# 0xMiden/miden-vm

Hardware: AMD Instinct MI355X
Metric: trace rows/sec proved (2^20-row trace, 96-bit sec) (higher is better)
Workload: dtype u64 (Goldilocks field, p = 2^64 - 2^32 + 1); 1 GPU; full proof of miden:20:51:8 (DummyMidenAir 2^20 x 51 + 8 EF aux), 96-bit production PCS params (blowup 8, FRI arity 4, 27 queries, PoW 4/12/16), Poseidon2 LMCS; trace resident in HBM, transcript on host; log_trace_rows=20, main_width=51, aux_width_ef=8, log_blowup=3, proof_bytes=137697, parallelism=1 GPU

## Files before the change

miden-vm_amd/csrc/deep.hip:

```cpp
#include "gl.cuh"
#include "kernels.hpp"

__global__ __launch_bounds__(256) void k_bary_weights(const u64* tw, int log_n, u64 g, e2 y0, e2 y1, u64* w0, u64* w1) {
  const size_t n = (size_t)1 << log_n;
  const size_t base = (size_t)blockIdx.x * 1024 + threadIdx.x;
  const size_t half = n >> 1;
  u64 xs[4], nrm[8], pre[8];
  e2 den[8];
#pragma unroll
  for (int k = 0; k < 4; k++) {
    size_t r = base + (size_t)k * 256;
    u64 x = 0;
    if (r < n) x = gl_mul(g, half ? (r < half ? tw[r] : gl_neg(tw[r - half])) : 1);
    xs[k] = x;
    den[2 * k] = e2_sub(y0, e2_make(x));
    den[2 * k + 1] = e2_sub(y1, e2_make(x));
  }
  u64 run = 1;
#pragma unroll
  for (int k = 0; k < 8; k++) {
    nrm[k] = gl_sub(gl_sqr(den[k].c0), gl_mul7(gl_sqr(den[k].c1)));
    pre[k] = run;
    run = gl_mul(run, nrm[k]);
  }
  u64 inv = gl_inv(run);
#pragma unroll
  for (int k = 7; k >= 0; k--) {
    u64 ni = gl_mul(inv, pre[k]);
    inv = gl_mul(inv, nrm[k]);
    size_t r = base + (size_t)(k >> 1) * 256;
    if (r < n) {
      u64 s = gl_mul(ni, xs[k >> 1]);
      u64* w = (k & 1) ? w1 : w0;
      w[2 * r] = gl_mul(den[k].c0, s);
      w[2 * r + 1] = gl_mul(gl_neg(den[k].c1), s);
    }
  }
}

static constexpr int OOD_ROWS_PER_BLOCK = 8192;
__global__ __launch_bounds__(256) void k_ood_partial(const u64* lde, int log_n, int log_blowup, const u64* w0, const u64* w1,
                                                     u64* partial, unsigned chunks) {
  __shared__ u64 red[4][256];
  const size_t n = (size_t)1 << log_n;
  const size_t col = blockIdx.y, chunk = blockIdx.x;
  const u64* f = lde + ((col << log_blowup) << log_n);
  const size_t r0 = chunk * OOD_ROWS_PER_BLOCK;
  const size_t r1 = r0 + OOD_ROWS_PER_BLOCK < n ? r0 + OOD_ROWS_PER_BLOCK : n;
  e2 a0 = e2_make(0), a1 = e2_make(0);
  for (size_t r = r0 + threadIdx.x; r < r1; r += 256) {
    u64 v = f[r];
    a0 = e2_add(a0, e2_mulf(e2{w0[2 * r], w0[2 * r + 1]}, v));
    a1 = e2_add(a1, e2_mulf(e2{w1[2 * r], w1[2 * r + 1]}, v));
  }
  red[0][threadIdx.x] = a0.c0; red[1][threadIdx.x] = a0.c1; red[2][threadIdx.x] = a1.c0; red[3][threadIdx.x] = a1.c1;
  __syncthreads();
  for (int s = 128; s > 0; s >>= 1) {
    if ((int)threadIdx.x < s) {
#pragma unroll
      for (int k = 0; k < 4; k++) red[k][threadIdx.x] = gl_add(red[k][threadIdx.x], red[k][threadIdx.x + s]);
    }
    __syncthreads();
  }
  if (threadIdx.x < 4) partial[(col * chunks + chunk) * 4 + threadIdx.x] = red[threadIdx.x][0];
}

void deep_ood_eval_batch(mh_ctx* c, std::vector<OodJob>& jobs, int log_blowup) {
  struct Weights {
    int log_n;
    size_t coset0;
    e2 y0, y1;
    DevBuf w0, w1;
  };
  std::vector<std::unique_ptr<Weights>> weights;
  struct Slot {
    size_t off = 0, ncol = 0;
    unsigned chunks = 0;
  };
  std::vector<Slot> slots(jobs.size());
  size_t total = 0;
  for (size_t k = 0; k < jobs.size(); k++) {
    OodJob& j = jobs[k];
    const LdeMatrix& m = *j.m;
    if (j.col_end > m.width) j.col_end = m.width;
    j.out0.assign(m.width, e2_make(0));
    j.out1.assign(m.width, e2_make(0));
    if (j.col_begin >= j.col_end) continue;
    const size_t n = (size_t)1 << m.log_n;
    slots[k].ncol = j.col_end - j.col_begin;
    slots[k].chunks = (unsigned)((n + OOD_ROWS_PER_BLOCK - 1) / OOD_ROWS_PER_BLOCK);
    slots[k].off = total;
    total += slots[k].ncol * slots[k].chunks * 4;
  }
  if (!total) return;
  DevBuf partial(total * 8), one;
  for (size_t k = 0; k < jobs.size(); k++) {
    if (!slots[k].ncol) continue;
    const OodJob& j = jobs[k];
    const LdeMatrix& m = *j.m;
    const int log_n = m.log_n;
    const size_t n = (size_t)1 << log_n;
    const u64 g = gl_mul(gl_lde_shift(log_n + log_blowup), gl_pow(gl_two_adic_generator(log_n + log_blowup), m.coset0));
    const u64* tw = log_n ? c->twiddles(log_n, false) : nullptr;
    if (!tw) {
      if (!one.p) {
        one.alloc(8);
        u64 v = 1;
        c->h2d(one.p, &v, 8);
      }
      tw = one.u();
    }
    ProfScope ps(c, "deep_ood_eval", (double)n * 8.0 * slots[k].ncol + 64.0 * n);
    Weights* w = nullptr;
    for (auto& cand : weights)
      if (cand->log_n == log_n && cand->coset0 == m.coset0 && e2_eq(cand->y0, j.y0) && e2_eq(cand->y1, j.y1)) w = cand.get();
    if (!w) {
      weights.emplace_back(new Weights{log_n, m.coset0, j.y0, j.y1, DevBuf(n * 16), DevBuf(n * 16)});
      w = weights.back().get();
      MH_LAUNCH(k_bary_weights, dim3((unsigned)((n + 1023) / 1024)), dim3(256), 0, c->stream, tw, log_n, g, j.y0, j.y1, w->w0.u(), w->w1.u());
    }
    MH_LAUNCH(k_ood_partial, dim3(slots[k].chunks, (unsigned)slots[k].ncol), dim3(256), 0, c->stream,
              m.lde.u() + ((j.col_begin << m.log_cosets) << log_n), log_n, m.log_cosets, w->w0.u(), w->w1.u(), partial.u() + slots[k].off,
              slots[k].chunks);
  }
  std::vector<u64> host(total);
  c->d2h(host.data(), partial.p, total * 8);
  for (size_t k = 0; k < jobs.size(); k++) {
    if (!slots[k].ncol) continue;
    OodJob& j = jobs[k];
    const LdeMatrix& m = *j.m;
    const int log_n = m.log_n;
    const size_t n = (size_t)1 << log_n;
    const u64 g = gl_mul(gl_lde_shift(log_n + log_blowup), gl_pow(gl_two_adic_generator(log_n + log_blowup), m.coset0));
    const u64 g_inv = gl_inv(g), n_inv = gl_inv((u64)n % GL_P);
    const e2 s0 = e2_mulf(e2_sub(e2_exp_pow2(e2_mulf(j.y0, g_inv), log_n), e2_make(1)), n_inv);
    const e2 s1 = e2_mulf(e2_sub(e2_exp_pow2(e2_mulf(j.y1, g_inv), log_n), e2_make(1)), n_inv);
    for (size_t col = 0; col < slots[k].ncol; col++) {
      e2 a0 = e2_make(0), a1 = e2_make(0);
      for (unsigned ch = 0; ch < slots[k].chunks; ch++) {
        const u64* p = host.data() + slots[k].off + (col * slots[k].chunks + ch) * 4;
        a0 = e2_add(a0, e2{p[0], p[1]});
        a1 = e2_add(a1, e2{p[2], p[3]});
      }
      j.out0[j.col_begin + col] = e2_mul(a0, s0);
      j.out1[j.col_begin + col] = e2_mul(a1, s1);
    }
  }
}
void deep_ood_eval_matrix(mh_ctx* c, const LdeMatrix& m, int log_blowup, e2 y0, e2 y1, std::vector<e2>& out0, std::vector<e2>& out1,
                          size_t col_begin, size_t col_end) {
  std::vector<OodJob> jobs(1);
  jobs[0].m = &m; jobs[0].y0 = y0; jobs[0].y1 = y1; jobs[0].col_begin = col_begin; jobs[0].col_end = col_end;
  deep_ood_eval_batch(c, jobs, log_blowup);
  out0.swap(jobs[0].out0);
  out1.swap(jobs[0].out1);
}

static constexpr int DEEP_MAX_MATS = 128;
static constexpr unsigned DEEP_FLUSH = 128;
#ifndef DEEP_UNROLL
#define DEEP_UNROLL 2
#endif
#ifndef DEEP_PTS_N
#define DEEP_PTS_N 1
#endif
static constexpr int DEEP_PTS = DEEP_PTS_N;
struct DeepMat {
  const u64* lde;
  u32 width, coef_off;
  int log_n;
};
struct DeepArgs {
  DeepMat m[DEEP_MAX_MATS];
  int n_mats, log_n, log_blowup;
  const u64* negc;
  const u64* tw;
  const u64* coset_x;
  e2 z0, z1, fred0, fred1, beta;
  u64* out;
};

__global__ __launch_bounds__(256) void k_deep_assemble(DeepArgs a) {
  const size_t N = (size_t)1 << a.log_n;
  const size_t j = blockIdx.y;
  const size_t base = (size_t)blockIdx.x * (256 * DEEP_PTS) + threadIdx.x;
  size_t r[DEEP_PTS];
#pragma unroll
  for (int k = 0; k < DEEP_PTS; k++) r[k] = base + (size_t)k * 256;
  e2 neg[DEEP_PTS];
  u64 w[DEEP_PTS][2][6];
#pragma unroll
  for (int k = 0; k < DEEP_PTS; k++) {
    neg[k] = e2_make(0);
#pragma unroll
    for (int e = 0; e < 2; e++)
#pragma unroll
      for (int i = 0; i < 6; i++) w[k][e][i] = 0;
  }
  auto flush = [&]() {
    const u64 C[6] = {1ULL, 1ULL << 22, 1ULL << 44, 1ULL << 32, 1ULL << 54, GL_EPS << 12};
#pragma unroll
    for (int k = 0; k < DEEP_PTS; k++) {
      u64 s0 = w[k][0][0], s1 = w[k][1][0];
#pragma unroll
      for (int i = 1; i < 6; i++) {
        s0 = gl_add(s0, gl_mul(w[k][0][i], C[i]));
        s1 = gl_add(s1, gl_mul(w[k][1][i], C[i]));
      }
      neg[k] = e2_add(neg[k], e2{s0, s1});
#pragma unroll
      for (int e = 0; e < 2; e++)
#pragma unroll
        for (int i = 0; i < 6; i++) w[k][e][i] = 0;
    }
  };
  u32 pending = 0;
#pragma unroll 1
  for (int mi = 0; mi < a.n_mats; mi++) {
    const DeepMat m = a.m[mi];
    const size_t nm_mask = ((size_t)1 << m.log_n) - 1;
    const u64* colp = m.lde + (j << m.log_n);
    const size_t cstride = (size_t)1 << (m.log_n + a.log_blowup);
#pragma unroll DEEP_UNROLL
    for (u32 cidx = 0; cidx < m.width; cidx++) {
      const u64 cf0 = a.negc[2 * (m.coef_off + cidx)], cf1 = a.negc[2 * (m.coef_off + cidx) + 1];
      u32 al[2][3];
#pragma unroll
      for (int i = 0; i < 3; i++) {
        al[0][i] = (u32)(cf0 >> (22 * i)) & 0x3FFFFFu;
        al[1][i] = (u32)(cf1 >> (22 * i)) & 0x3FFFFFu;
      }
#pragma unroll
      for (int k = 0; k < DEEP_PTS; k++) {
        if (r[k] < N) {
          const u64 v = colp[r[k] & nm_mask];
          const u32 v0 = (u32)v, v1 = (u32)(v >> 32);
#pragma unroll
          for (int e = 0; e < 2; e++) {
            w[k][e][0] += (u64)al[e][0] * v0;
            w[k][e][1] += (u64)al[e][1] * v0;
            w[k][e][2] += (u64)al[e][2] * v0;
            w[k][e][3] += (u64)al[e][0] * v1;
            w[k][e][4] += (u64)al[e][1] * v1;
            w[k][e][5] += (u64)al[e][2] * v1;
          }
        }
      }
      colp += cstride;
      if (++pending == DEEP_FLUSH) {
        flush();
        pending = 0;
      }
    }
  }
  flush();
  const size_t half = N >> 1;
  const u64 cx = a.coset_x[j];
  e2 den[2 * DEEP_PTS];
  u64 nrm[2 * DEEP_PTS], pre[2 * DEEP_PTS];
#pragma unroll
  for (int k = 0; k < DEEP_PTS; k++) {
    u64 x = 0;
    if (r[k] < N) x = gl_mul(cx, half ? (r[k] < half ? a.tw[r[k]] : gl_neg(a.tw[r[k] - half])) : 1);
    den[2 * k] = e2_sub(a.z0, e2_make(x));
    den[2 * k + 1] = e2_sub(a.z1, e2_make(x));
  }
  u64 run = 1;
#pragma unroll
  for (int k = 0; k < 2 * DEEP_PTS; k++) {
    nrm[k] = gl_sub(gl_sqr(den[k].c0), gl_mul7(gl_sqr(den[k].c1)));
    pre[k] = run;
    run = gl_mul(run, nrm[k]);
  }
  u64 inv = gl_inv(run);
  e2 qinv[2 * DEEP_PTS];
#pragma unroll
  for (int k = 2 * DEEP_PTS - 1; k >= 0; k--) {
    u64 ni = gl_mul(inv, pre[k]);
    inv = gl_mul(inv, nrm[k]);
    qinv[k] = e2{gl_mul(den[k].c0, ni), gl_mul(gl_neg(den[k].c1), ni)};
  }
#pragma unroll
  for (int k = 0; k < DEEP_PTS; k++) {
    if (r[k] < N) {
      e2 v = e2_mul(qinv[2 * k], e2_add(a.fred0, neg[k]));
      v = e2_add(v, e2_mul(e2_mul(a.beta, qinv[2 * k + 1]), e2_add(a.fred1, neg[k])));
      ulonglong2* o = reinterpret_cast<ulonglong2*>(a.out + 2 * ((j << a.log_n) + r[k]));
      *o = make_ulonglong2(v.c0, v.c1);
    }
  }
}

void deep_assemble(mh_ctx* c, const std::vector<const LdeMatrix*>& mats, const std::vector<u32>& coef_off, int log_n, int log_blowup,
                   const std::vector<e2>& negc, e2 z0, e2 z1, e2 fred0, e2 fred1, e2 beta, u64* out) {
  MH_REQUIRE(mats.size() <= (size_t)DEEP_MAX_MATS, "too many committed matrices for one DEEP pass");
  const int lbl = mats[0]->log_cosets;
  const size_t coset0 = mats[0]->coset0;
  for (auto* m : mats) MH_REQUIRE(m->log_cosets == lbl && m->coset0 == coset0, "internal: matrices cover different cosets");
  const size_t N = (size_t)1 << log_n, B = (size_t)1 << lbl;
  const int L = log_n + log_blowup;
  std::vector<u64> blob;
  for (e2 v : negc) { blob.push_back(v.c0); blob.push_back(v.c1); }
  const size_t o_cx = blob.size();
  const u64 g = gl_lde_shift(L), wK = gl_two_adic_generator(L);
  u64 x = gl_mul(g, gl_pow(wK, coset0));
  for (size_t j = 0; j < B; j++) {
    blob.push_back(x);
    x = gl_mul(x, wK);
  }
  DevBuf dblob(blob.size() * 8), one;
  c->h2d(dblob.p, blob.data(), blob.size() * 8);
  const u64* tw = log_n ? c->twiddles(log_n, false) : nullptr;
  if (!tw) {
    one.alloc(8);
    u64 v = 1;
    c->h2d(one.p, &v, 8);
    tw = one.u();
  }
  DeepArgs a{};
  double bytes = 16.0 * N * B;
  for (size_t i = 0; i < mats.size(); i++) {
    a.m[i] = DeepMat{mats[i]->lde.u(), (u32)mats[i]->width, coef_off[i], mats[i]->log_n};
    bytes += 8.0 * (double)mats[i]->width * (double)(((size_t)1 << mats[i]->log_n) << lbl);
  }
  a.n_mats = (int)mats.size();
  a.log_n = log_n; a.log_blowup = lbl;
  a.negc = dblob.u(); a.tw = tw; a.coset_x = dblob.u() + o_cx;
  a.z0 = z0; a.z1 = z1; a.fred0 = fred0; a.fred1 = fred1; a.beta = beta; a.out = out;
  {
    ProfScope ps(c, "deep_assemble", bytes);
    MH_LAUNCH(k_deep_assemble, dim3((unsigned)((N + 256 * DEEP_PTS - 1) / (256 * DEEP_PTS)), (unsigned)B), dim3(256), 0, c->stream, a);
  }
  HIP_CHECK(hipStreamSynchronize(c->stream));
}
```

miden-vm_amd/csrc/kernels.hpp:

```cpp
#pragma once
#include "../../include/midenhip.h"
#include "ctx.hpp"
#include <functional>
#include <vector>

void launch_transpose_rm_to_cm(mh_ctx* c, const u64* in_rowmajor, u64* out_colmajor, size_t n, size_t w, hipStream_t stream = nullptr);
void ntt_inverse_dif_inplace(mh_ctx* c, u64* cols, size_t n_cols, int log_n);
void ntt_inverse_dif(mh_ctx* c, const u64* src, u64* dst, size_t n_cols, int log_n);
void ntt_forward_cosets(mh_ctx* c, const u64* coef_br, size_t n_cols, int log_n, const std::vector<u64>& bases, u64* out, size_t out_col_stride = 0,
                        size_t group_cols = 0);
void lde_columns(mh_ctx* c, const u64* cols_in, size_t n_cols, int log_n, u64 in_shift, const std::vector<u64>& out_shifts,
                 u64* out, u64* scratch);
void lde_coefficients(mh_ctx* c, const u64* cols_in, size_t n_cols, int log_n, u64* coef_br);
void lde_forward_group(mh_ctx* c, const u64* coef_br, size_t n_cols, int log_n, u64 in_shift, const std::vector<u64>& group_shifts,
                       u64* out, size_t out_col_stride);

struct mh_trace {
  mh_ctx* ctx;
  int log_n;
  size_t width;
  DevBuf cols;
  hipEvent_t ready = nullptr;
  mutable DevBuf staging;
  size_t col_group = 0;
  std::vector<hipEvent_t> col_ready;
  ~mh_trace() {
    if (ready) (void)hipEventSynchronize(ready);
    else if ((staging.p || !col_ready.empty()) && ctx && ctx->copy_stream) (void)hipStreamSynchronize(ctx->copy_stream);
    for (hipEvent_t e : col_ready)
      if (e != ready) (void)hipEventDestroy(e);
    if (ready) (void)hipEventDestroy(ready);
  }
};
void trace_wait_ready(mh_ctx* c, const mh_trace* t);
mh_trace* trace_upload_cols_async(mh_ctx* c, const u64* colmajor, int log_n, size_t width);

struct LdeMatrix {
  int log_n;
  size_t width;
  DevBuf lde;
  int log_cosets = 0;
  size_t coset0 = 0;
};

struct mh_comm;
struct Dist {
  const mh_comm* comm = nullptr;
  int rank = 0, world = 1, logG = 0;
  bool on() const { return world > 1; }
  void all_to_all(mh_ctx* c, const void* send, void* recv, size_t bytes_per_peer) const;
  void all_gather(mh_ctx* c, const void* send, void* recv, size_t bytes_per_rank) const;
  void all_reduce_sum(mh_ctx* c, u64* buf, size_t n) const;
};

struct mh_tree {
  mh_ctx* ctx;
  int log_blowup;
  int log_height;
  int lmcs = 0;
  SaltArgs salt;
  std::vector<LdeMatrix> mats;
  DevBuf fri_layer;
  int fri_log_rows = -1;
  int fri_log_arity = 0;
  int fri_log_cosets = 0;
  size_t fri_coset0 = 0;
  int shard_logG = 0, shard_rank = 0;
  std::vector<u64> cap;
  DevBuf nodes;
  std::vector<size_t> layer_off;
  u64 root[4];
  size_t node_slot(int d, size_t p) const {
    int cbits = d - (log_height - log_blowup);
    if (cbits <= 0) return p;
    size_t j = p & (((size_t)1 << cbits) - 1), r = p >> cbits;
    return (j << (log_height - log_blowup)) + r;
  }
};

void poseidon2_permute_device(mh_ctx* c, u64* states_soa, size_t n);
double poseidon2_register_rate(mh_ctx* c);
void lmcs_build_tree(mh_ctx* c, mh_tree* t);
void lmcs_hash_leaves(mh_ctx* c, const std::vector<LdeMatrix>& mats, int lb, u64* digests, const SaltArgs* salt = nullptr);
void lmcs_hash_leaves_range(mh_ctx* c, const std::vector<LdeMatrix>& mats, int lb, u64* digests, size_t q_begin, size_t q_count,
                            const SaltArgs* salt = nullptr);
void lmcs_salt_assign(mh_ctx* c, mh_tree* t);
const SaltArgs* lmcs_salt_of(const mh_tree* t);
void lmcs_salt_rows(mh_ctx* c, const SaltArgs& salt, const u64* rows, size_t n_rows, u64* out);
bool lmcs_leaves_rangeable(mh_ctx* c, const std::vector<LdeMatrix>& mats);
void lmcs_alloc_layers(mh_tree* t, int log_height);
u64* lmcs_leaf_layer(mh_tree* t);
void lmcs_compress_layers(mh_ctx* c, mh_tree* t);
void lmcs_open(mh_ctx* c, const mh_tree* t, const std::vector<size_t>& sorted_unique_idx, size_t alignment,
               std::vector<u64>& fields, std::vector<u64>& commitments, const Dist* dist = nullptr);
struct OpenPlan {
  size_t first = 0, n_fields = 0, n = 0;
  std::vector<std::pair<size_t, const u64*>> cap_fill;
  DevBuf salt_rows;
};
OpenPlan lmcs_open_plan(const mh_tree* t, const std::vector<size_t>& idx, size_t alignment, const Dist* dist, std::vector<const u64*>& ptrs);
void lmcs_open_run(mh_ctx* c, const std::vector<const u64*>& ptrs, const Dist* dist, std::vector<u64>& host);
void lmcs_open_take(const OpenPlan& plan, std::vector<u64>& host, std::vector<u64>& fields, std::vector<u64>& commitments);
void lmcs_build_sharded(mh_ctx* c, mh_tree* t, const Dist& dist, const u64* local_digests, int log_rows);
void lmcs_host_compress(int lmcs, const u64* pair, u64* out);
void lmcs_host_compress_level(int lmcs, const u64* children, size_t n_out, u64* out);
bool p2_host_simd_available();
void p2_host_compress8(const u64* pairs, int n, u64* out);
void p2_host_permute8(u64* states );
std::vector<std::pair<int, size_t>> lmcs_missing_siblings(const std::vector<size_t>& sorted_unique_idx, int depth);

std::vector<u64> coset_shifts(int log_n, int lb);
mh_trace* trace_upload(mh_ctx* c, const u64* rowmajor, int log_n, size_t width);
mh_trace* trace_upload_async(mh_ctx* c, const u64* rowmajor, int log_n, size_t width);
mh_trace* trace_zeros(mh_ctx* c, int log_n, size_t width);
mh_tree* commit_traces(mh_ctx* c, const std::vector<const mh_trace*>& traces, int log_blowup);
LdeMatrix lde_trace_cosets(mh_ctx* c, const mh_trace* tr, int lb, size_t first, size_t count);
struct mh_air;
#include "gl.cuh"
void quotient_eval_accumulate(mh_ctx* c, const mh_air* air, const LdeMatrix& main, const LdeMatrix& aux, const LdeMatrix* prep,
                              int log_blowup, int log_d,
                              const std::vector<u64>& publics, const std::vector<e2>& randomness, const std::vector<e2>& aux_values,
                              e2 alpha, const u64* acc_in, int log_n_prev, e2 beta, u64* acc_out);
void quotient_upsample_accumulate(mh_ctx* c, const u64* q_small, int log_n, int log_blowup, int log_dj, int log_d, const u64* acc_in,
                                  int log_n_prev, e2 beta, u64* acc_out, size_t t_first, size_t n_local);
struct OodJob {
  const LdeMatrix* m = nullptr;
  e2 y0, y1;
  size_t col_begin = 0, col_end = ~(size_t)0;
  std::vector<e2> out0, out1;
};
void deep_ood_eval_batch(mh_ctx* c, std::vector<OodJob>& jobs, int log_blowup);
void deep_ood_eval_matrix(mh_ctx* c, const LdeMatrix& m, int log_blowup, e2 y0, e2 y1, std::vector<e2>& out0, std::vector<e2>& out1,
                          size_t col_begin = 0, size_t col_end = (size_t)-1);
void deep_assemble(mh_ctx* c, const std::vector<const LdeMatrix*>& mats, const std::vector<uint32_t>& coef_off, int log_n, int log_blowup,
                   const std::vector<e2>& negc, e2 z0, e2 z1, e2 fred0, e2 fred1, e2 beta, u64* out);
void fri_leaf_hash(mh_ctx* c, const u64* ev, int log_rows, int cbits, int log_arity, u64* digests, const SaltArgs* salt = nullptr);
void fri_fold(mh_ctx* c, const u64* ev, int log_rows, int cbits, int cbits_global, size_t coset0, int log_arity, e2 beta, u64* out);
void fri_to_natural(mh_ctx* c, const u64* ev, int log_rows, int cbits, u64* out);
u64 fri_grind(mh_ctx* c, const u64 st[12], const u64* in, int n_in, int bits);
u64 fri_grind_bytes(mh_ctx* c, int lmcs, const std::vector<uint8_t>& prefix, int bits);

struct mh_lookup;
mh_trace* lookup_build_aux(mh_ctx* c, const mh_lookup* lk, const mh_trace* main, const mh_trace* prep, const std::vector<e2>& randomness,
                           e2* acc_final);
void lookup_planes(mh_ctx* c, const mh_lookup* lk, const mh_trace* main, const mh_trace* prep, const std::vector<e2>& randomness, DevBuf& planes);

void constraint_fold_trace_domain(mh_ctx* c, const mh_air* air, const mh_trace* main, const mh_trace* aux, const mh_trace* prep,
                                  const u64* inv_first, const u64* inv_last, const std::vector<u64>& publics, const std::vector<e2>& randomness,
                                  const std::vector<e2>& aux_values, e2 alpha, u64* acc);
int check_statement(mh_ctx* c, int n_airs, mh_air* const* airs, mh_trace* const* traces, const mh_trace* const* preps, const u64* publics,
                    size_t n_publics, const u64 challenger_state[12], const u64* pre_observe, size_t n_pre, mh_external_assertions ext,
                    void* ext_user, const char* const* names, int flags, mh_check_entry* out, size_t cap, size_t* n_entries);
std::vector<e2> debug_challenges(const u64 challenger_state[12], const u64* pre_observe, size_t n_pre, int n_airs, mh_trace* const* traces,
                                 size_t count);
size_t compact_rows(mh_ctx* c, const u32* flags, size_t n, u64* rows);

struct BoundaryPush {
  e2 denom;
  int sign;
};
bool precompile_session_boundary(bool fixed_uints, e2 alpha, e2 beta, std::vector<BoundaryPush>& out);
int balance_statement(mh_ctx* c, int n_airs, mh_air* const* airs, mh_trace* const* traces, const mh_trace* const* preps,
                      const u64 challenger_state[12], const u64* pre_observe, size_t n_pre,
                      const std::function<bool(const std::vector<e2>&, std::vector<BoundaryPush>&)>& boundary, const char* const* names, int flags,
                      mh_balance_entry* entries, size_t entry_cap, size_t* n_entries, mh_balance_push* pushes, size_t push_cap, size_t* n_pushes);
```

miden-vm_amd/csrc/prover.hip:

```cpp
#include "../../include/midenhip.h"
#include "air.hpp"
#include "air_jit.hpp"
#include "challenger.hpp"
#include "ctx.hpp"
#include "gl.cuh"
#include "kernels.hpp"
#include "poseidon2.cuh"
#include <algorithm>
#include <chrono>
#include <cstring>
#include <thread>
#include <memory>
#include <numeric>

std::vector<u64> coset_shifts(int log_n, int lb) {
  u64 g = gl_lde_shift(log_n + lb);
  u64 wk = gl_two_adic_generator(log_n + lb);
  std::vector<u64> s((size_t)1 << lb);
  u64 x = g;
  for (auto& v : s) {
    v = x;
    x = gl_mul(x, wk);
  }
  return s;
// ... 368 lines not shown
    L = log_N + lb;
    MH_REQUIRE(L <= 32, "LDE order exceeds the field's two-adicity");
    N = (size_t)1 << log_N;
    for (int i = 0; i < n_airs; i++) logD = std::max(logD, airs[i]->log_quotient_degree);
    MH_REQUIRE(logD <= lb, "constraint degree too high for the blowup");
    D = (size_t)1 << logD;
    publics.assign(publics_in, publics_in + n_publics);
    if (dist.on()) {
      MH_REQUIRE(dist.logG <= lb, "more ranks than cosets");
      for (int i = 0; i < n_airs; i++) MH_REQUIRE(lhs[i] >= dist.logG, "trace shorter than the number of ranks");
    }
    lbl = lb - dist.logG;
    B_loc = (size_t)1 << lbl;
    coset0 = (size_t)dist.rank * B_loc;
    D_loc = chunks_on_rank(logD);
    D_slot = std::max<size_t>(1, D >> dist.logG);
    prep_of.assign(n_airs, -1);
    int n_prep = 0;
    for (int j = 0; j < n_airs; j++) {
      const mh_air* a = airs[order[j]];
      if (!a->preprocessed_width) continue;
      MH_REQUIRE(a->prep_tree, "AIR declares preprocessed columns but no preprocessed tree is attached");
      MH_REQUIRE(!prep_tree || prep_tree == a->prep_tree, "all AIRs must share one preprocessed tree");
      prep_tree = a->prep_tree;
      MH_REQUIRE(a->prep_index == n_prep, "preprocessed matrices must be committed in proof order (ascending height, ties by instance)");
      MH_REQUIRE((size_t)a->prep_index < prep_tree->mats.size(), "preprocessed matrix index out of range");
      const LdeMatrix& m = prep_tree->mats[a->prep_index];
      MH_REQUIRE(m.width == a->preprocessed_width, "preprocessed matrix width differs from the AIR's declaration");
      MH_REQUIRE(m.log_n == lhs[order[j]], "preprocessed matrix height differs from the main trace height");
      prep_of[j] = n_prep++;
    }
    if (prep_tree) {
      MH_REQUIRE(prep_tree->log_blowup == lb, "preprocessed tree was committed under a different blowup");
      MH_REQUIRE(prep_tree->shard_logG == dist.logG && (!dist.on() || prep_tree->shard_rank == dist.rank),
                 "preprocessed tree was committed for a different sharding (use mh_commit_traces_sharded with the same communicator)");
      MH_REQUIRE((int)prep_tree->mats.size() == n_prep, "preprocessed tree holds matrices no AIR declares");
      MH_REQUIRE(prep_tree->lmcs == c->lmcs, "the preprocessed (setup) tree was committed with another LMCS hasher than this context's");
      MH_REQUIRE(prep_tree->salt.n == c->salt.n, "the preprocessed (setup) tree was committed with another salt width than this context's (mh_ctx_set_salt)");
    }
    rounds = fri_num_rounds(pp, L);
    stage = 1;
  }
  size_t alignment() const { return c->lmcs == MH_LMCS_BLAKE3 ? 1 : (c->lmcs == MH_LMCS_KECCAK ? 17 : 8); }
  size_t al(size_t w) const {
    const size_t a = alignment();
    return (w + a - 1) / a * a;
  }
  size_t ood_width() const {
    size_t w = 0;
    for (int i = 0; i < n_airs; i++)
      w += al(airs[i]->main_width) + al(2 * airs[i]->aux_width) + (airs[i]->preprocessed_width ? al(airs[i]->preprocessed_width) : 0);
    return w + al(2 * D);
  }
  size_t num_aux_values() const {
    size_t k = 0;
    for (int i = 0; i < n_airs; i++) k += airs[i]->num_aux_values;
    return k;
  }
  size_t final_poly_len() const { return (size_t)1 << std::max(0, L - rounds * pp.log_folding_arity - lb); }
  int lmcs0 = 0;
  int salt0 = 0;
  void expect(int s, const char* what) {
    MH_REQUIRE(stage == s, std::string("session call out of protocol order: ") + what);
    MH_REQUIRE(c->lmcs == lmcs0, "the context's LMCS hasher changed during the session");
    MH_REQUIRE(c->salt.n == salt0, "the context's salt width changed during the session");
  }

  void commit_main(u64 root[4]) {
    expect(1, "commit_main");
    ProfScope span(c, "span:commit to main traces");
    std::vector<const mh_trace*> po;
    for (int j = 0; j < n_airs; j++) po.push_back(traces[order[j]]);
    main_tree.reset(commit_traces_dist(c, po, lb, dist));
    memcpy(root, main_tree->root, 32);
    stage = 2;
  }
  void commit_aux(const std::vector<e2>& rnd, mh_aux_builder cb, void* user, u64 root[4], std::vector<e2>& aux_values_out) {
    expect(2, "commit_aux");
    ProfScope span(c, "span:build aux traces + commit to aux traces");
    MH_REQUIRE(rnd.size() == max_rand, "wrong number of randomness elements");
    randomness = rnd;
    std::vector<u64> rand_flat;
    for (e2 r : randomness) { rand_flat.push_back(r.c0); rand_flat.push_back(r.c1); }
    if (rand_flat.empty()) rand_flat.push_back(0);
    std::vector<std::unique_ptr<mh_trace>> aux_tr(n_airs);
    struct HostScratch {
      mh_ctx* c;
      std::vector<std::pair<void*, size_t>> bufs;
      ~HostScratch() {
        if (!bufs.empty() && c->copy_stream) (void)hipStreamSynchronize(c->copy_stream);
        for (auto& b : bufs) c->host_give(b.first, b.second);
      }
    } scratch{c, {}};
    aux_vals.assign(n_airs, {});
    for (int i = 0; i < n_airs; i++) {
      const mh_air* a = airs[i];
      const size_t n = (size_t)1 << lhs[i], w = 2 * a->aux_width;
      aux_vals[i].assign(a->num_aux_values, e2_make(0));
      if (a->lookup) {
        e2 fin;
        MH_REQUIRE(!a->lookup->preprocessed_width || a->prep_raw, "the lookup program reads preprocessed columns: attach the preprocessed matrix too");
        aux_tr[i].reset(lookup_build_aux(c, a->lookup, traces[i], a->prep_raw, randomness, &fin));
        aux_vals[i][0] = fin;
      } else if (cb) {
        std::vector<u64> vals(2 * std::max<size_t>(1, a->num_aux_values), 0);
        const size_t bytes = std::max<size_t>(8, n * w * 8);
        u64* host = static_cast<u64*>(c->host_take(bytes));
        scratch.bufs.emplace_back(host, bytes);
        memset(host, 0, n * w * 8);
        int rc = cb(user, i, rand_flat.data(), host, vals.data());
        MH_REQUIRE(rc == 0, "aux trace builder / external assertion failed");
        for (size_t k = 0; k < a->num_aux_values; k++) aux_vals[i][k] = e2{gl_canon(vals[2 * k]), gl_canon(vals[2 * k + 1])};
        aux_tr[i].reset(w ? trace_upload_async(c, host, lhs[i], w) : trace_upload(c, host, lhs[i], w));
      } else {
        aux_tr[i].reset(trace_zeros(c, lhs[i], w));
      }
    }
    std::vector<const mh_trace*> po;
    for (int j = 0; j < n_airs; j++) po.push_back(aux_tr[order[j]].get());
    aux_tree.reset(commit_traces_dist(c, po, lb, dist));
    memcpy(root, aux_tree->root, 32);
    aux_values_out.clear();
    for (int j = 0; j < n_airs; j++)
      for (e2 v : aux_vals[order[j]]) aux_values_out.push_back(v);
    stage = 3;
  }
  void commit_quotient(e2 alpha, e2 beta, u64 root[4]) {
    expect(3, "commit_quotient");
    ProfScope span(c, "span:evaluate constraints + commit to quotient poly chunks");
    DevBuf acc;
    int log_n_prev = 0;
    for (int j = 0; j < n_airs; j++) {
      const mh_air* a = airs[order[j]];
      const int ln = lhs[order[j]];
      DevBuf out(std::max<size_t>(8, ((size_t)2 * D_loc << ln) * 8));
      std::vector<e2> rnd(randomness.begin(), randomness.begin() + a->num_randomness);
      const int logDj = a->log_quotient_degree;
      const LdeMatrix* prep = prep_of[j] >= 0 ? &prep_tree->mats[prep_of[j]] : nullptr;
      if (logDj == logD) {
        if (D_loc)
          quotient_eval_accumulate(c, a, main_tree->mats[j], aux_tree->mats[j], prep, lb, logD, publics, rnd, aux_vals[order[j]], alpha,
                                   j ? acc.u() : nullptr, log_n_prev, beta, out.u());
      } else {
        const size_t dj_loc = chunks_on_rank(logDj), dj_slot = std::max<size_t>(1, ((size_t)1 << logDj) >> dist.logG);
        const size_t chunk_words = (size_t)2 << ln;
        DevBuf mine(dj_slot * chunk_words * 8);
        if (dj_loc)
          quotient_eval_accumulate(c, a, main_tree->mats[j], aux_tree->mats[j], prep, lb, logDj, publics, rnd, aux_vals[order[j]], alpha,
                                   nullptr, 0, beta, mine.u());
        DevBuf small;
        if (dist.on()) {
          small.alloc(((size_t)2 << (logDj + ln)) * 8);
          DevBuf all((size_t)dist.world * dj_slot * chunk_words * 8);
          dist.all_gather(c, mine.u(), all.p, dj_slot * chunk_words * 8);
          for (size_t t = 0; t < ((size_t)1 << logDj); t++)
            HIP_CHECK(hipMemcpyAsync(small.u() + t * chunk_words, all.u() + gathered_chunk(logDj, dj_slot, t) * chunk_words, chunk_words * 8,
                                     hipMemcpyDeviceToDevice, c->stream));
          c->sync();
        } else {
          small = std::move(mine);
        }
        quotient_upsample_accumulate(c, small.u(), ln, lb, logDj, logD, j ? acc.u() : nullptr, log_n_prev, beta, out.u(),
                                     first_chunk_on_rank(logD), D_loc);
      }
      acc = std::move(out);
      log_n_prev = ln;
    }
    quot_tree.reset(new mh_tree());
    quot_tree->ctx = c; quot_tree->log_blowup = lb;
    LdeMatrix qm;
    qm.log_n = log_N; qm.width = 2 * D;
    qm.log_cosets = lbl; qm.coset0 = coset0;
    qm.lde.alloc(N * B_loc * 2 * D * 8);
    const u64 g = gl_lde_shift(L);
    const u64 wJ = gl_two_adic_generator(log_N + logD);
    const std::vector<u64> all_outs = coset_shifts(log_N, lb);
    DevBuf gathered, slot_buf;
    const u64* coef = acc.u();
    if (D_loc) {
      ProfScope ps(c, "lde", (double)N * 2 * D_loc * 8.0);
      ntt_inverse_dif_inplace(c, acc.u(), 2 * D_loc, log_N);
    }
    if (dist.on()) {
      const u64* mine = acc.u();
      if (!D_loc) {
        slot_buf.alloc(2 * D_slot * N * 8);
        HIP_CHECK(hipMemsetAsync(slot_buf.p, 0, 2 * D_slot * N * 8, c->stream));
        mine = slot_buf.u();
      }
      gathered.alloc((size_t)dist.world * 2 * D_slot * N * 8);
      dist.all_gather(c, mine, gathered.p, 2 * D_slot * N * 8);
      coef = gathered.u();
    }
    {
      ProfScope ps(c, "lde", (double)B_loc * N * 2 * D * 8.0);
      std::vector<u64> bases(D * B_loc);
      bool contiguous = true;
      for (size_t t = 0; t < D; t++) {
        const u64 in_inv = gl_inv(gl_mul(g, gl_pow(wJ, t)));
        for (size_t zc = 0; zc < B_loc; zc++) bases[t * B_loc + zc] = gl_mul(all_outs[coset0 + zc], in_inv);
        contiguous = contiguous && (dist.on() ? gathered_chunk(logD, D_slot, t) : t) == t;
      }
      static const int grouped = [] { const char* e = getenv("MH_QUOTIENT_LDE_GROUPED"); return e ? atoi(e) : 1; }();
      if (grouped && contiguous && D > 1) {
        ntt_forward_cosets(c, coef, 2 * D, log_N, bases, qm.lde.u(), 0, 2);
      } else {
        for (size_t t = 0; t < D; t++) {
          const size_t src_chunk = dist.on() ? gathered_chunk(logD, D_slot, t) : t;
          const std::vector<u64> bt(bases.begin() + t * B_loc, bases.begin() + (t + 1) * B_loc);
          ntt_forward_cosets(c, coef + 2 * src_chunk * N, 2, log_N, bt, qm.lde.u() + 2 * t * B_loc * N);
        }
      }
    }
    quot_tree->mats.push_back(std::move(qm));
    if (dist.on()) {
      DevBuf dig((B_loc << log_N) * 32);
      lmcs_hash_leaves(c, quot_tree->mats, lbl, dig.u());
      lmcs_build_sharded(c, quot_tree.get(), dist, dig.u(), log_N);
    } else {
      lmcs_salt_assign(c, quot_tree.get());
      lmcs_build_tree(c, quot_tree.get());
    }
    memcpy(root, quot_tree->root, 32);
    stage = 4;
  }
  bool ood_point_ok(e2 cand) const {
    if (e2_is_zero(cand)) return false;
    if (e2_eq(e2_exp_pow2(cand, log_N), e2_make(1))) return false;
    const u64 g_inv = gl_inv(gl_lde_shift(L));
    if (e2_eq(e2_exp_pow2(e2_mulf(cand, g_inv), L), e2_make(1))) return false;
    return true;
  }
  void ood(e2 zp) {
    expect(4, "ood");
    ProfScope span(c, "span:evaluate at OOD points");
    MH_REQUIRE(ood_point_ok(zp), "OOD point lies on the trace domain or the LDE coset");
    z = zp;
    z_next = e2_mulf(z, gl_two_adic_generator(log_N));
    mats.clear(); coef_off.clear();
    if (prep_tree)
      for (auto& m : prep_tree->mats) mats.push_back(&m);
    for (auto& m : main_tree->mats) mats.push_back(&m);
    for (auto& m : aux_tree->mats) mats.push_back(&m);
    mats.push_back(&quot_tree->mats[0]);
    W = 0;
    for (auto* m : mats) {
      coef_off.push_back((u32)W);
      W += al(m->width);
    }
    ev0.assign(W, e2_make(0));
    ev1.assign(W, e2_make(0));
    std::vector<OodJob> jobs(mats.size());
    for (size_t i = 0; i < mats.size(); i++) {
      const int lift = log_N - mats[i]->log_n;
      size_t cb = 0, ce = mats[i]->width;
      if (dist.on()) {
        const size_t per = (mats[i]->width + dist.world - 1) / dist.world;
        cb = std::min(mats[i]->width, per * dist.rank);
        ce = std::min(mats[i]->width, cb + per);
      }
      jobs[i].m = mats[i];
      jobs[i].y0 = e2_exp_pow2(z, lift);
      jobs[i].y1 = e2_exp_pow2(z_next, lift);
      jobs[i].col_begin = cb;
      jobs[i].col_end = ce;
    }
    deep_ood_eval_batch(c, jobs, lb);
    for (size_t i = 0; i < mats.size(); i++)
      for (size_t k = 0; k < jobs[i].out0.size(); k++) {
        ev0[coef_off[i] + k] = jobs[i].out0[k];
        ev1[coef_off[i] + k] = jobs[i].out1[k];
      }
    if (dist.on() && W) {
      std::vector<u64> flat(4 * W);
      for (size_t i = 0; i < W; i++) {
        flat[4 * i] = ev0[i].c0; flat[4 * i + 1] = ev0[i].c1; flat[4 * i + 2] = ev1[i].c0; flat[4 * i + 3] = ev1[i].c1;
      }
      DevBuf d(flat.size() * 8);
      c->h2d(d.p, flat.data(), flat.size() * 8);
      dist.all_reduce_sum(c, d.u(), flat.size());
      c->d2h(flat.data(), d.p, flat.size() * 8);
      for (size_t i = 0; i < W; i++) {
        ev0[i] = e2{flat[4 * i], flat[4 * i + 1]};
        ev1[i] = e2{flat[4 * i + 2], flat[4 * i + 3]};
      }
    }
    stage = 5;
  }
  void deep(e2 alpha_d, e2 beta_d) {
    expect(5, "deep");
    ProfScope span(c, "span:DEEP quotient");
    e2 fred0 = e2_make(0), fred1 = e2_make(0);
    for (size_t i = 0; i < W; i++) {
      fred0 = e2_add(e2_mul(fred0, alpha_d), ev0[i]);
      fred1 = e2_add(e2_mul(fred1, alpha_d), ev1[i]);
    }
    std::vector<e2> negc(W);
    e2 pw = e2_make(GL_P - 1);
    for (size_t i = W; i-- > 0;) {
      negc[i] = pw;
      pw = e2_mul(pw, alpha_d);
    }
    layer.alloc((N << lbl) * 16);
    deep_assemble(c, mats, coef_off, log_N, lb, negc, z, z_next, fred0, fred1, beta_d, layer.u());
    log_rows = log_N; cbits = lb; cb_loc = lbl; fri_c0 = coset0;
    sharded = dist.on();
    stage = 6;
  }
  void fri_commit(u64 root[4]) {
    expect(6, "fri_commit");
    ProfScope span(c, "span:FRI round commit");
    MH_REQUIRE((int)fri_trees.size() < rounds && !round_committed, "no FRI round left to commit");
    const int la = pp.log_folding_arity;
    if (sharded && log_rows - la < dist.logG) {
      DevBuf full(((size_t)1 << (log_rows + cbits)) * 16);
      dist.all_gather(c, layer.p, full.p, ((size_t)1 << (log_rows + cb_loc)) * 16);
      layer = std::move(full);
      cb_loc = cbits;
      fri_c0 = 0;
      sharded = false;
    }
    if (log_rows < la) {
      MH_REQUIRE(!sharded, "internal: sharded FRI layer shorter than the arity");
      DevBuf nat(((size_t)1 << (log_rows + cbits)) * 16);
      fri_to_natural(c, layer.u(), log_rows, cbits, nat.u());
      c->sync();
      layer = std::move(nat);
      log_rows += cbits;
      cbits = 0;
      cb_loc = 0;
    }
    std::unique_ptr<mh_tree> t(new mh_tree());
    t->ctx = c; t->log_blowup = cbits;
    t->fri_log_rows = log_rows; t->fri_log_arity = la;
    t->fri_log_cosets = cb_loc; t->fri_coset0 = fri_c0;
    if (sharded) {
      DevBuf dig(((size_t)1 << (log_rows - la + cb_loc)) * 32);
      fri_leaf_hash(c, layer.u(), log_rows, cb_loc, la, dig.u());
      lmcs_build_sharded(c, t.get(), dist, dig.u(), log_rows - la);
    } else {
      lmcs_alloc_layers(t.get(), log_rows + cbits - la);
      lmcs_salt_assign(c, t.get());
      fri_leaf_hash(c, layer.u(), log_rows, cbits, la, lmcs_leaf_layer(t.get()), lmcs_salt_of(t.get()));
      lmcs_compress_layers(c, t.get());
    }
    memcpy(root, t->root, 32);
    fri_trees.push_back(std::move(t));
    round_committed = true;
  }
  void fri_fold_round(e2 fb) {
    expect(6, "fri_fold");
    ProfScope span(c, "span:FRI fold");
    MH_REQUIRE(round_committed, "fold before the round's commitment");
    const int la = pp.log_folding_arity;
    DevBuf next(((size_t)1 << (log_rows + cb_loc - la)) * 16);
    fri_fold(c, layer.u(), log_rows, cb_loc, cbits, fri_c0, la, fb, next.u());
    fri_trees.back()->fri_layer = std::move(layer);
    layer = std::move(next);
    log_rows -= la;
    round_committed = false;
  }
  void fri_final(std::vector<e2>& desc) {
    expect(6, "fri_final");
    ProfScope span(c, "span:idft final poly");
    MH_REQUIRE((int)fri_trees.size() == rounds && !round_committed, "FRI rounds not finished");
    const int logn_f = log_rows + cbits;
    const int log_fpd = std::max(0, logn_f - lb);
    const size_t fpd = (size_t)1 << log_fpd;
    const size_t n_loc = (size_t)1 << (log_rows + cb_loc);
    std::vector<u64> host(2 * n_loc);
    c->d2h(host.data(), layer.p, n_loc * 16);
    std::vector<e2> vals(fpd);
    u64 s_shift = 1;
    if (sharded) {
      MH_REQUIRE(cbits == lb && fpd == ((size_t)1 << log_rows), "internal: final layer shape");
      for (size_t r = 0; r < fpd; r++) vals[r] = e2{host[2 * r], host[2 * r + 1]};
      s_shift = gl_pow(gl_two_adic_generator(logn_f), fri_c0);
    } else {
      for (size_t r = 0; r < fpd; r++) {
        size_t i = r << (logn_f - log_fpd);
        size_t slot = ((i & (((size_t)1 << cbits) - 1)) << log_rows) + (i >> cbits);
        vals[r] = e2{host[2 * slot], host[2 * slot + 1]};
      }
    }
    const u64 w_inv = gl_inv(gl_two_adic_generator(log_fpd)), n_inv = gl_inv((u64)fpd);
    const u64 s_inv = gl_inv(s_shift);
    std::vector<e2> coef(fpd);
    u64 sk = 1;
    for (size_t k = 0; k < fpd; k++) {
      e2 s = e2_make(0);
      u64 wk = gl_pow(w_inv, k), x = 1;
      for (size_t r = 0; r < fpd; r++) {
        s = e2_add(s, e2_mulf(vals[r], x));
        x = gl_mul(x, wk);
      }
      coef[k] = e2_mulf(s, gl_mul(n_inv, sk));
      sk = gl_mul(sk, s_inv);
    }
    desc.assign(coef.rbegin(), coef.rend());
    layer.release();
    stage = 7;
  }
  void open(std::vector<size_t> idx, std::vector<u64>& fields, std::vector<u64>& commitments) {
    expect(7, "open");
    ProfScope span(c, "span:query phase");
    std::sort(idx.begin(), idx.end());
    idx.erase(std::unique(idx.begin(), idx.end()), idx.end());
    for (size_t i : idx) MH_REQUIRE(i < ((size_t)1 << L), "query index out of range");
    std::vector<const u64*> ptrs;
    std::vector<OpenPlan> plans;
    if (prep_tree) {
      std::vector<size_t> pidx(idx);
      const size_t mask = ((size_t)1 << (prep_tree->log_height + prep_tree->shard_logG)) - 1;
      for (auto& i : pidx) i &= mask;
      std::sort(pidx.begin(), pidx.end());
      pidx.erase(std::unique(pidx.begin(), pidx.end()), pidx.end());
      plans.push_back(lmcs_open_plan(prep_tree, pidx, alignment(), &dist, ptrs));
    }
    for (const mh_tree* t : {main_tree.get(), aux_tree.get(), quot_tree.get()}) plans.push_back(lmcs_open_plan(t, idx, alignment(), &dist, ptrs));
    int depth = L;
    for (auto& t : fri_trees) {
      depth -= pp.log_folding_arity;
      const size_t mask = ((size_t)1 << depth) - 1;
      for (auto& i : idx) i &= mask;
      std::sort(idx.begin(), idx.end());
      idx.erase(std::unique(idx.begin(), idx.end()), idx.end());
      plans.push_back(lmcs_open_plan(t.get(), idx, 1, &dist, ptrs));
    }
    std::vector<u64> host;
    lmcs_open_run(c, ptrs, &dist, host);
    for (const OpenPlan& plan : plans) {
      std::vector<u64> f, cm;
      lmcs_open_take(plan, host, f, cm);
      fields.insert(fields.end(), f.begin(), f.end());
      commitments.insert(commitments.end(), cm.begin(), cm.end());
    }
    stage = 8;
  }
};

static void do_grind(mh_ctx* c, HostTranscript& tr, int bits) {
  if (bits == 0) {
    tr.fields.push_back(0);
    return;
  }
  if (bits <= 5 && tr.ch.hash == MH_LMCS_POSEIDON2 && p2_host_simd_available()) {
    HostChallenger& ch = tr.ch;
    const size_t k = ch.in.size() + 1;
    u64 base[12];
    for (int i = 0; i < 12; i++) base[i] = ch.st[i];
    for (size_t i = 0; i + 1 < k; i++) base[i] = ch.in[i];
    for (size_t i = k; i < 8; i++) base[i] = 0;
    base[8] = gl_add(base[8], (u64)k);
    const u64 mask = ((u64)1 << bits) - 1;
    for (u64 w0 = 0;; w0 += 8) {
      u64 states[8][12];
      for (int j = 0; j < 8; j++) {
        memcpy(states[j], base, 96);
        states[j][k - 1] = w0 + (u64)j;
      }
      p2_host_permute8(&states[0][0]);
      for (int j = 0; j < 8; j++)
        if (((states[j][7] & 0xFFFFFFFFULL) & mask) == 0) {
          MH_REQUIRE(ch.check_witness(bits, w0 + (u64)j), "internal: vectorised PoW witness rejected by the challenger");
          tr.fields.push_back(w0 + (u64)j);
          return;
        }
    }
  }
  if (bits <= 5) {
    for (u64 w = 0;; w++) {
      HostChallenger trial = tr.ch;
      if (trial.check_witness(bits, w)) {
        tr.ch = trial;
        tr.fields.push_back(w);
        return;
      }
    }
  }
  u64 w = tr.ch.bytes() ? fri_grind_bytes(c, tr.ch.hash, tr.ch.bin, bits)
                        : fri_grind(c, tr.ch.st, tr.ch.in.data(), (int)tr.ch.in.size(), bits);
  MH_REQUIRE(tr.ch.check_witness(bits, w), "internal: device PoW witness rejected by the host challenger");
  tr.fields.push_back(w);
}

static void prove_impl(mh_ctx* c, const mh_pcs_params& pp, int n_airs, mh_air* const* airs_in, mh_trace* const* traces_in,
                       const u64* publics_in, size_t n_publics, const u64 init_state[12], const u64* pre_observe, size_t n_pre,
                       mh_aux_builder cb, void* user, mh_proof& proof, const Dist& dist) {
  mh_session s;
  s.begin(c, pp, n_airs, airs_in, traces_in, publics_in, n_publics, dist);
  HostTranscript tr;
  tr.ch.hash = c->lmcs;
  tr.ch.init_from_state(init_state);
  for (size_t i = 0; i < n_pre; i++) tr.ch.observe_framing(pre_observe[i]);
  tr.ch.observe((u64)n_airs);
  for (int i = 0; i < n_airs; i++) tr.ch.observe((u64)s.lhs[i]);

  u64 root[4];
  s.commit_main(root);
  tr.send_commitment(root);
  std::vector<e2> rnd;
  for (size_t i = 0; i < s.max_rand; i++) rnd.push_back(tr.ch.sample_ef());
  std::vector<e2> aux_values;
  s.commit_aux(rnd, cb, user, root, aux_values);
  tr.send_commitment(root);
  for (e2 v : aux_values) tr.send_ef(v);
  const e2 alpha = tr.ch.sample_ef();
  const e2 beta = tr.ch.sample_ef();
  s.commit_quotient(alpha, beta, root);
  tr.send_commitment(root);
  e2 z;
  do {
    z = tr.ch.sample_ef();
  } while (!s.ood_point_ok(z));
  s.ood(z);
  for (e2 v : s.ev0) tr.send_ef(v);
  for (e2 v : s.ev1) tr.send_ef(v);
  do_grind(c, tr, pp.deep_pow_bits);
  const e2 alpha_d = tr.ch.sample_ef();
  const e2 beta_d = tr.ch.sample_ef();
  s.deep(alpha_d, beta_d);
  for (int r = 0; r < s.rounds; r++) {
    s.fri_commit(root);
    tr.send_commitment(root);
    do_grind(c, tr, pp.folding_pow_bits);
    s.fri_fold_round(tr.ch.sample_ef());
  }
  std::vector<e2> final_poly;
  s.fri_final(final_poly);
  for (e2 v : final_poly) tr.send_ef(v);
  do_grind(c, tr, pp.query_pow_bits);
  std::vector<size_t> idx;
  for (int i = 0; i < pp.num_queries; i++) idx.push_back(tr.ch.sample_bits(s.L));
  std::vector<u64> f, cm;
  s.open(idx, f, cm);
  tr.hint_fields(f);
  tr.hint_commitments(cm);
  tr.ch.finalize(proof.digest);
  for (int i = 0; i < n_airs; i++) proof.log_trace_heights.push_back((uint8_t)s.lhs[i]);
  proof.fields = std::move(tr.fields);
  for (auto& d : tr.commitments) proof.commitments.insert(proof.commitments.end(), d.begin(), d.end());
}

#define MH_TRY(ctx_expr) mh_ctx* _c = (ctx_expr); PoolScope _ps(_c); try {
#define MH_CATCH                                                   \
  }                                                                \
  catch (const MhError& e) {                                       \
    if (_c) _c->err = e.what();                                    \
    return e.code;                                                 \
  }                                                                \
  catch (const std::exception& e) {                                \
    if (_c) _c->err = e.what();                                    \
    return MH_ERR_INTERNAL;                                        \
  }                                                                \
  return MH_OK;

extern "C" {

int mh_air_load(mh_ctx* c, const uint64_t* blob, size_t n_words, mh_air** out) {
  MH_TRY(c)
  MH_REQUIRE(c && blob && out, "null argument");
  HIP_CHECK(hipSetDevice(c->device));
  *out = mh_air::load(c, blob, n_words);
  MH_CATCH
}
void mh_air_free(mh_air* a) {
  if (!a) return;
  (void)hipSetDevice(a->ctx->device);
  PoolScope ps(a->ctx);
  delete a;
}
int mh_air_log_quotient_degree(const mh_air* a) { return a ? a->log_quotient_degree : -1; }
int mh_jit_precompile(const uint64_t* blob, size_t n_words, int* n_chunks) {
  try {
    if (!blob) return MH_ERR_INVALID;
    const int k = jit_precompile_blob(blob, n_words);
    if (n_chunks) *n_chunks = k;
    return MH_OK;
  } catch (const MhError& e) {
    return e.code;
  } catch (const std::exception&) {
    return MH_ERR_INTERNAL;
  }
}
int mh_lookup_load(mh_ctx* c, const uint64_t* blob, size_t n_words, mh_lookup** out) {
  MH_TRY(c)
  MH_REQUIRE(c && blob && out, "null argument");
  HIP_CHECK(hipSetDevice(c->device));
  *out = mh_lookup::load(c, blob, n_words);
  MH_CATCH
}
void mh_lookup_free(mh_lookup* l) {
  if (!l) return;
  (void)hipSetDevice(l->ctx->device);
  PoolScope ps(l->ctx);
  delete l;
}
int mh_air_attach_lookup(mh_air* a, const mh_lookup* l) {
  MH_TRY(a ? a->ctx : nullptr)
  MH_REQUIRE(a, "null argument");
  if (l) {
    MH_REQUIRE(l->main_width == a->main_width, "lookup program and AIR disagree on the trace width");
    MH_REQUIRE(l->num_aux_cols() == a->aux_width, "lookup program and AIR disagree on the number of aux columns");
    MH_REQUIRE(a->num_aux_values == 1, "a LogUp AIR commits exactly one aux value (the accumulator's final)");
    MH_REQUIRE(l->num_randomness <= a->num_randomness, "lookup program needs more challenges than the AIR samples");
    MH_REQUIRE(l->preprocessed_width == 0 || l->preprocessed_width == a->preprocessed_width,
               "lookup program and AIR disagree on the preprocessed width");
// ... 446 lines not shown
```

Baseline: 23.41 million trace rows/s.

## Evaluate DEEP quotient on one coset and extend via LDE

The DEEP quotient is now computed only on the first coset, written as two base-field planes. It is then interpolated and re-evaluated on all blowup cosets with the existing column LDE path, and finally interleaved into the FRI layer layout. This avoids reading every committed LDE matrix on all cosets, which was the main memory cost of DEEP assembly. In exchange it adds a small NTT round trip, extra scratch buffers and an interleave pass. It also relies on the DEEP combination having degree below the trace length. An environment variable restores the old all-coset path.

```diff
diff --git a/miden-vm_amd/csrc/deep.hip b/miden-vm_amd/csrc/deep.hip
--- a/miden-vm_amd/csrc/deep.hip
+++ b/miden-vm_amd/csrc/deep.hip
@@ -180,6 +180,7 @@
   u64* out;
 };
 
+template <bool PLANES>
 __global__ __launch_bounds__(256) void k_deep_assemble(DeepArgs a) {
   const size_t N = (size_t)1 << a.log_n;
   const size_t j = blockIdx.y;
@@ -285,14 +286,25 @@
     if (r[k] < N) {
       e2 v = e2_mul(qinv[2 * k], e2_add(a.fred0, neg[k]));
       v = e2_add(v, e2_mul(e2_mul(a.beta, qinv[2 * k + 1]), e2_add(a.fred1, neg[k])));
-      ulonglong2* o = reinterpret_cast<ulonglong2*>(a.out + 2 * ((j << a.log_n) + r[k]));
-      *o = make_ulonglong2(v.c0, v.c1);
-    }
-  }
+      if constexpr (PLANES) {
+        a.out[r[k]] = v.c0;
+        a.out[N + r[k]] = v.c1;
+      } else {
+        ulonglong2* o = reinterpret_cast<ulonglong2*>(a.out + 2 * ((j << a.log_n) + r[k]));
+        *o = make_ulonglong2(v.c0, v.c1);
+      }
+    }
+  }
+}
+
+__global__ __launch_bounds__(256) void k_deep_interleave(const u64* __restrict__ planes, size_t n, u64* __restrict__ out) {
+  const size_t i = (size_t)blockIdx.x * 256 + threadIdx.x;
+  if (i >= n) return;
+  *reinterpret_cast<ulonglong2*>(out + 2 * i) = make_ulonglong2(planes[i], planes[n + i]);
 }
 
 void deep_assemble(mh_ctx* c, const std::vector<const LdeMatrix*>& mats, const std::vector<u32>& coef_off, int log_n, int log_blowup,
-                   const std::vector<e2>& negc, e2 z0, e2 z1, e2 fred0, e2 fred1, e2 beta, u64* out) {
+                   const std::vector<e2>& negc, e2 z0, e2 z1, e2 fred0, e2 fred1, e2 beta, u64* out, bool one_coset) {
   MH_REQUIRE(mats.size() <= (size_t)DEEP_MAX_MATS, "too many committed matrices for one DEEP pass");
   const int lbl = mats[0]->log_cosets;
   const size_t coset0 = mats[0]->coset0;
@@ -317,19 +329,36 @@
     c->h2d(one.p, &v, 8);
     tw = one.u();
   }
+  MH_REQUIRE(!one_coset || (lbl >= 1 && log_n >= DEEP_ONE_COSET_MIN_LOG_N), "internal: one-coset DEEP assemble needs two cosets to extend to");
+  const size_t Ba = one_coset ? 1 : B;
   DeepArgs a{};
-  double bytes = 16.0 * N * B;
+  double bytes = 16.0 * N * Ba;
   for (size_t i = 0; i < mats.size(); i++) {
     a.m[i] = DeepMat{mats[i]->lde.u(), (u32)mats[i]->width, coef_off[i], mats[i]->log_n};
-    bytes += 8.0 * (double)mats[i]->width * (double)(((size_t)1 << mats[i]->log_n) << lbl);
+    bytes += 8.0 * (double)mats[i]->width * (double)(((size_t)1 << mats[i]->log_n) * Ba);
   }
   a.n_mats = (int)mats.size();
   a.log_n = log_n; a.log_blowup = lbl;
   a.negc = dblob.u(); a.tw = tw; a.coset_x = dblob.u() + o_cx;
   a.z0 = z0; a.z1 = z1; a.fred0 = fred0; a.fred1 = fred1; a.beta = beta; a.out = out;
+  const dim3 grid((unsigned)((N + 256 * DEEP_PTS - 1) / (256 * DEEP_PTS)), (unsigned)Ba);
+  if (!one_coset) {
+    ProfScope ps(c, "deep_assemble", bytes);
+    MH_LAUNCH(k_deep_assemble<false>, grid, dim3(256), 0, c->stream, a);
+    HIP_CHECK(hipStreamSynchronize(c->stream));
+    return;
+  }
+  DevBuf planes(2 * N * 8), scratch(2 * N * 8), ext(2 * B * N * 8);
+  a.out = planes.u();
   {
     ProfScope ps(c, "deep_assemble", bytes);
-    MH_LAUNCH(k_deep_assemble, dim3((unsigned)((N + 256 * DEEP_PTS - 1) / (256 * DEEP_PTS)), (unsigned)B), dim3(256), 0, c->stream, a);
+    MH_LAUNCH(k_deep_assemble<true>, grid, dim3(256), 0, c->stream, a);
+  }
+  {
+    ProfScope ps(c, "deep_extend", 16.0 * N + 3.0 * 16.0 * N * B);
+    const std::vector<u64> shifts(blob.begin() + o_cx, blob.begin() + o_cx + B);
+    lde_columns(c, planes.u(), 2, log_n, shifts[0], shifts, ext.u(), scratch.u());
+    MH_LAUNCH(k_deep_interleave, dim3((unsigned)((B * N + 255) / 256)), dim3(256), 0, c->stream, ext.u(), B * N, out);
   }
   HIP_CHECK(hipStreamSynchronize(c->stream));
 }
diff --git a/miden-vm_amd/csrc/kernels.hpp b/miden-vm_amd/csrc/kernels.hpp
--- a/miden-vm_amd/csrc/kernels.hpp
+++ b/miden-vm_amd/csrc/kernels.hpp
@@ -132,8 +132,9 @@
 void deep_ood_eval_batch(mh_ctx* c, std::vector<OodJob>& jobs, int log_blowup);
 void deep_ood_eval_matrix(mh_ctx* c, const LdeMatrix& m, int log_blowup, e2 y0, e2 y1, std::vector<e2>& out0, std::vector<e2>& out1,
                           size_t col_begin = 0, size_t col_end = (size_t)-1);
+static constexpr int DEEP_ONE_COSET_MIN_LOG_N = 2;
 void deep_assemble(mh_ctx* c, const std::vector<const LdeMatrix*>& mats, const std::vector<uint32_t>& coef_off, int log_n, int log_blowup,
-                   const std::vector<e2>& negc, e2 z0, e2 z1, e2 fred0, e2 fred1, e2 beta, u64* out);
+                   const std::vector<e2>& negc, e2 z0, e2 z1, e2 fred0, e2 fred1, e2 beta, u64* out, bool one_coset);
 void fri_leaf_hash(mh_ctx* c, const u64* ev, int log_rows, int cbits, int log_arity, u64* digests, const SaltArgs* salt = nullptr);
 void fri_fold(mh_ctx* c, const u64* ev, int log_rows, int cbits, int cbits_global, size_t coset0, int log_arity, e2 beta, u64* out);
 void fri_to_natural(mh_ctx* c, const u64* ev, int log_rows, int cbits, u64* out);
diff --git a/miden-vm_amd/csrc/prover.hip b/miden-vm_amd/csrc/prover.hip
--- a/miden-vm_amd/csrc/prover.hip
+++ b/miden-vm_amd/csrc/prover.hip
@@ -694,7 +694,9 @@
       pw = e2_mul(pw, alpha_d);
     }
     layer.alloc((N << lbl) * 16);
-    deep_assemble(c, mats, coef_off, log_N, lb, negc, z, z_next, fred0, fred1, beta_d, layer.u());
+    const char* all_env = getenv("MH_DEEP_ALL_COSETS");
+    const bool one_coset = !(all_env && atoi(all_env)) && lbl >= 1 && log_N >= DEEP_ONE_COSET_MIN_LOG_N;
+    deep_assemble(c, mats, coef_off, log_N, lb, negc, z, z_next, fred0, fred1, beta_d, layer.u(), one_coset);
     log_rows = log_N; cbits = lb; cb_loc = lbl; fri_c0 = coset0;
     sharded = dist.on();
     stage = 6;
```

New measurement: 24.05 million trace rows/s (median of 6 runs). +2.7%, better.
